# nasa/PROTEUS

Measured on AMD Instinct MI355X. Metric: Mpixels/sec DSWx classify (3660^2 7-band HLS tiles), higher is better.
Workload: dtype int16+f64

## Files before the change

### proteus_amd/csrc/dswx_outline.hip

```cpp
#include <hip/hip_runtime.h>
#include <cstdio>
#include <cstring>
#include <vector>

#include "dswx_host.h"
#include "dswx_body_rule.h"
#include "dswx_outline_rule.h"

namespace {

typedef u32x4 __attribute__((aligned(16))) out_u32x4;

constexpr int OUT_BLOCK = 256;
constexpr int OUT_PPT = 16;
constexpr int OUT_WAVES = OUT_BLOCK / 64;
constexpr int OUT_CHUNK = DSWX_OUTLINE_CHUNK;
static_assert(DSWX_OUTLINE_CHUNK == DSWX_BODY_CHUNK && DSWX_OUTLINE_SCAN_STEP == DSWX_BODY_SCAN_STEP, "the scan of the body table");
static_assert(OUT_BLOCK * OUT_PPT == OUT_CHUNK && DSWX_OUTLINE_SCAN_STEP == OUT_BLOCK, "a workgroup's threads cover a chunk");
constexpr int64_t OUT_MAX_PIXELS = 1LL << 30;
constexpr int64_t OUT_MAX_CAP = 1LL << 31;
constexpr unsigned OUT_CORNER = 0x80000000u;
constexpr int OUT_MAX_ROUNDS = 31;
constexpr unsigned OUT_NO_RING = 0xFFFFFFFFu;

struct OutlineInfo {
    unsigned long long E;
    unsigned long long R;
    unsigned ok;
    unsigned fin;
    unsigned flag[OUT_MAX_ROUNDS + 1];
};
static_assert(sizeof(OutlineInfo) <= 256, "the info block of a tile");

struct OutlineLayout {
    unsigned long long cap;
    unsigned long long base, mask, st0, st1, acc, part, info, per_tile;
    unsigned chunks_p, chunks_e, rounds, acc_blocks;
};
inline unsigned long long up16(unsigned long long v) { return (v + 15ull) & ~15ull; }
OutlineLayout outline_layout(int64_t max_edges, int64_t height, int64_t width) {
    OutlineLayout l = {};
    const unsigned long long n = (unsigned long long)(height * width);
    l.cap = (unsigned long long)max_edges < 4ull * n ? (unsigned long long)max_edges : 4ull * n;
    l.chunks_p = (unsigned)((n + OUT_CHUNK - 1) / OUT_CHUNK);
    l.chunks_e = (unsigned)((l.cap + OUT_CHUNK - 1) / OUT_CHUNK);
    while ((1ull << l.rounds) < l.cap) ++l.rounds;
    const unsigned long long rings = l.cap / 4ull;
    l.acc_blocks = (unsigned)((rings + OUT_BLOCK - 1) / OUT_BLOCK);
    unsigned long long at = 0;
    l.base = at, at += up16(4ull * n);
    l.mask = at, at += up16(n);
    l.st0 = at, at += 16ull * l.cap;
    l.st1 = at, at += 16ull * l.cap;
    l.acc = at, at += 16ull * rings;
    l.part = at, at += up16(8ull * l.chunks_e);
    l.info = at, at += 256ull;
    l.per_tile = at;
    return l;
}

struct OutlineArgs {
    const unsigned* ids;
    unsigned char* work;
    OutlineLayout l;
    unsigned long long n_elems;
    long long n_tiles;
    unsigned height, width;
    int connectivity;
    unsigned round;
    unsigned long long max_edges, max_rings;
    unsigned* chain;
    unsigned* rings;
    unsigned long long* head;
};

struct DevIds {
    const unsigned* p;
    __device__ __forceinline__ unsigned operator()(uint64_t i) const { return p[i]; }
};

__device__ __forceinline__ unsigned char* tile_work(const OutlineArgs& a, long long t) { return a.work + (unsigned long long)t * a.l.per_tile; }
__device__ __forceinline__ unsigned* w_base(const OutlineArgs& a, long long t) { return reinterpret_cast<unsigned*>(tile_work(a, t) + a.l.base); }
__device__ __forceinline__ unsigned char* w_mask(const OutlineArgs& a, long long t) { return tile_work(a, t) + a.l.mask; }
__device__ __forceinline__ out_u32x4* w_state(const OutlineArgs& a, long long t, unsigned which) {
    return reinterpret_cast<out_u32x4*>(tile_work(a, t) + (which ? a.l.st1 : a.l.st0));
}
__device__ __forceinline__ unsigned long long* w_acc(const OutlineArgs& a, long long t) {
    return reinterpret_cast<unsigned long long*>(tile_work(a, t) + a.l.acc);
}
__device__ __forceinline__ unsigned* w_part(const OutlineArgs& a, long long t) { return reinterpret_cast<unsigned*>(tile_work(a, t) + a.l.part); }
__device__ __forceinline__ OutlineInfo* w_info(const OutlineArgs& a, long long t) { return reinterpret_cast<OutlineInfo*>(tile_work(a, t) + a.l.info); }

__device__ __forceinline__ unsigned out_wave_sum(unsigned v) {
#pragma unroll
    for (int o = 32; o > 0; o >>= 1) v += __shfl_xor(v, o);
    return v;
}
__device__ __forceinline__ unsigned out_wave_scan(unsigned v, unsigned lane) {
#pragma unroll
    for (int o = 1; o < 64; o <<= 1) {
        const unsigned u = __shfl_up(v, o);
        if (lane >= (unsigned)o) v += u;
    }
    return v;
}
__device__ __forceinline__ long long out_shfl_up64(long long v, int o) {
    const unsigned lo = __shfl_up((unsigned)(unsigned long long)v, o), hi = __shfl_up((unsigned)((unsigned long long)v >> 32), o);
    return (long long)(((unsigned long long)hi << 32) | lo);
}

__device__ __forceinline__ unsigned out_block_scan(unsigned v, unsigned* wtot, unsigned* total) {
    const unsigned lane = threadIdx.x & 63u, wave = threadIdx.x >> 6;
    const unsigned inc = out_wave_scan(v, lane);
    if (lane == 63u) wtot[wave] = inc;
    __syncthreads();
    unsigned before = 0, sum = 0;
#pragma unroll
    for (int w = 0; w < OUT_WAVES; ++w) {
        if ((unsigned)w < wave) before += wtot[w];
        sum += wtot[w];
    }
    __syncthreads();
    *total = sum;
    return before + inc - v;
}

__device__ __forceinline__ unsigned out_succ_number(const OutlineArgs& a, const unsigned* ids, const unsigned* base, const unsigned char* mask,
                                                    unsigned x, unsigned y, unsigned d, unsigned v) {
    const OutlineEdge s = outline_succ(DevIds{ids}, (int64_t)x, (int64_t)y, d, (int64_t)a.width, (int64_t)a.height, v, a.connectivity);
    const unsigned long long q = (unsigned long long)s.y * a.width + (unsigned long long)s.x;
    const unsigned e = base[q] + __popc((unsigned)mask[q] & ((1u << s.d) - 1u));
    return e | (s.d != d ? OUT_CORNER : 0u);
}

__global__ __launch_bounds__(OUT_BLOCK) void dswx_outline_count_k(const OutlineArgs a) {
    __shared__ unsigned wtot[OUT_WAVES];
    const unsigned long long chunk_first = (unsigned long long)blockIdx.x * OUT_CHUNK;
    const unsigned long long first = chunk_first + (unsigned long long)threadIdx.x * OUT_PPT;
    const unsigned lane = threadIdx.x & 63u, wave = threadIdx.x >> 6;
    for (long long t = blockIdx.y; t < a.n_tiles; t += gridDim.y) {
        const unsigned* const ids = a.ids + (unsigned long long)t * a.n_elems;
        unsigned char* const mask = w_mask(a, t);
        unsigned c = 0;
        if (first < a.n_elems) {
            unsigned y = (unsigned)(first / a.width), x = (unsigned)(first - (unsigned long long)y * a.width);
            unsigned m[OUT_PPT];
#pragma unroll
            for (int i = 0; i < OUT_PPT; ++i) {
                m[i] = 0u;
                if (first + i < a.n_elems) {
                    const unsigned v = ids[first + i];
                    if (v) m[i] = outline_mask(DevIds{ids}, (int64_t)x, (int64_t)y, (int64_t)a.width, (int64_t)a.height, v);
                    c += __popc(m[i]);
                    if (++x == a.width) x = 0u, ++y;
                }
            }
            if (first + OUT_PPT <= a.n_elems) {
                u32x4 q;
#pragma unroll
                for (int w = 0; w < 4; ++w) q[w] = m[4 * w] | (m[4 * w + 1] << 8) | (m[4 * w + 2] << 16) | (m[4 * w + 3] << 24);
                *reinterpret_cast<out_u32x4*>(mask + first) = q;
            } else {
#pragma unroll
                for (int i = 0; i < OUT_PPT; ++i)
                    if (first + i < a.n_elems) mask[first + i] = (unsigned char)m[i];
            }
        }
        c = out_wave_sum(c);
        if (lane == 0) wtot[wave] = c;
        __syncthreads();
        if (threadIdx.x == 0) {
            unsigned sum = 0;
#pragma unroll
            for (int w = 0; w < OUT_WAVES; ++w) sum += wtot[w];
            w_base(a, t)[chunk_first] = sum;
        }
        __syncthreads();
    }
}

__global__ __launch_bounds__(OUT_BLOCK) void dswx_outline_scan_k(const OutlineArgs a) {
    __shared__ unsigned wtot[OUT_WAVES];
    for (long long t = blockIdx.x; t < a.n_tiles; t += gridDim.x) {
        unsigned* const b = w_base(a, t);
        unsigned long long carry = 0;
        for (unsigned first = 0; first < a.l.chunks_p; first += DSWX_OUTLINE_SCAN_STEP) {
            const unsigned c = first + threadIdx.x;
            const unsigned val = c < a.l.chunks_p ? b[(unsigned long long)c * OUT_CHUNK] : 0u;
            unsigned total;
            const unsigned before = out_block_scan(val, wtot, &total);
            if (c < a.l.chunks_p) b[(unsigned long long)c * OUT_CHUNK] = (unsigned)carry + before;
            carry += total;
        }
        OutlineInfo* const info = w_info(a, t);
        const bool ok = carry <= a.max_edges;
        if (threadIdx.x <= OUT_MAX_ROUNDS) info->flag[threadIdx.x] = 0u;
        if (threadIdx.x == 0) {
            info->E = carry;
            info->R = 0ull;
            info->ok = ok ? 1u : 0u;
            info->fin = 0u;
        }
        if (a.head && threadIdx.x < DSWX_OUTLINE_HEAD_WORDS) {
            const unsigned w = threadIdx.x;
            a.head[(unsigned long long)t * DSWX_OUTLINE_HEAD_WORDS + w] =
                w == OUTLINE_HEAD_E ? carry : w == OUTLINE_HEAD_WRITTEN ? (ok ? carry : 0ull) : w == OUTLINE_HEAD_OVERFLOW ? (ok ? 0ull : 1ull) : 0ull;
        }
    }
}

__global__ __launch_bounds__(OUT_BLOCK) void dswx_outline_base_k(const OutlineArgs a) {
    __shared__ unsigned wtot[OUT_WAVES];
    __shared__ unsigned chunk_base;
    const unsigned long long chunk_first = (unsigned long long)blockIdx.x * OUT_CHUNK;
    const unsigned long long first = chunk_first + (unsigned long long)threadIdx.x * OUT_PPT;
    for (long long t = blockIdx.y; t < a.n_tiles; t += gridDim.y) {
        if (!w_info(a, t)->ok) continue;
        unsigned* const b = w_base(a, t);
        const unsigned char* const mask = w_mask(a, t);
        unsigned m[OUT_PPT], c = 0;
#pragma unroll
        for (int i = 0; i < OUT_PPT; ++i) {
            m[i] = first + i < a.n_elems ? (unsigned)mask[first + i] : 0u;
            c += __popc(m[i]);
        }
        if (threadIdx.x == 0) chunk_base = b[chunk_first];
        unsigned total;
        const unsigned before = out_block_scan(c, wtot, &total);
        unsigned e = chunk_base + before;
#pragma unroll
        for (int i = 0; i < OUT_PPT; ++i)
            if (first + i < a.n_elems) {
                b[first + i] = e;
                e += __popc(m[i]);
            }
        __syncthreads();
    }
}

__global__ __launch_bounds__(OUT_BLOCK) void dswx_outline_emit_k(const OutlineArgs a) {
    const unsigned long long first = (unsigned long long)blockIdx.x * OUT_CHUNK + (unsigned long long)threadIdx.x * OUT_PPT;
    if (first >= a.n_elems) return;
    for (long long t = blockIdx.y; t < a.n_tiles; t += gridDim.y) {
        if (!w_info(a, t)->ok) continue;
        const unsigned* const ids = a.ids + (unsigned long long)t * a.n_elems;
        const unsigned* const b = w_base(a, t);
        const unsigned char* const mask = w_mask(a, t);
        out_u32x4* const st = w_state(a, t, 0u);
        unsigned y = (unsigned)(first / a.width), x = (unsigned)(first - (unsigned long long)y * a.width);
        for (int i = 0; i < OUT_PPT && first + i < a.n_elems; ++i) {
            const unsigned p = (unsigned)(first + i), m = mask[p];
            if (m) {
                const unsigned v = ids[p];
                unsigned e = b[p];
                for (unsigned d = 0; d < 4u; ++d)
                    if ((m >> d) & 1u) {
                        st[e] = u32x4{out_succ_number(a, ids, b, mask, x, y, d, v), e, 0u, 4u * p + d};
                        ++e;
                    }
            }
            if (++x == a.width) x = 0u, ++y;
        }
    }
}

__global__ __launch_bounds__(OUT_BLOCK) void dswx_outline_jump_k(const OutlineArgs a) {
    const unsigned long long e = (unsigned long long)blockIdx.x * OUT_BLOCK + threadIdx.x;
    const unsigned k = a.round;
    for (long long t = blockIdx.y; t < a.n_tiles; t += gridDim.y) {
        OutlineInfo* const info = w_info(a, t);
        if (!info->ok || (k > 0u && !info->flag[k - 1u])) continue;
        if ((unsigned long long)blockIdx.x * OUT_BLOCK >= info->E) continue;
        const out_u32x4* const src = w_state(a, t, k & 1u);
        out_u32x4* const dst = w_state(a, t, (k + 1u) & 1u);
        if (blockIdx.x == 0 && threadIdx.x == 0) info->fin = (k + 1u) & 1u;
        bool take = false;
        if (e < info->E) {
            const u32x4 s = src[e];
            const u32x4 o = src[s.x & ~OUT_CORNER];
            take = o.y < s.y;
            dst[e] = u32x4{(o.x & ~OUT_CORNER) | (s.x & OUT_CORNER), take ? o.y : s.y, take ? (1u << k) + o.z : s.z, s.w};
        }
        if (__any(take) && (threadIdx.x & 63u) == 0u) info->flag[k] = 1u;
    }
}

__global__ __launch_bounds__(OUT_BLOCK) void dswx_outline_ring_count_k(const OutlineArgs a) {
    __shared__ unsigned wtot[OUT_WAVES];
    const unsigned long long first = (unsigned long long)blockIdx.x * OUT_CHUNK + (unsigned long long)threadIdx.x * OUT_PPT;
    for (long long t = blockIdx.y; t < a.n_tiles; t += gridDim.y) {
        const OutlineInfo* const info = w_info(a, t);
        if (!info->ok) continue;
        const unsigned long long E = info->E;
        const out_u32x4* const st = w_state(a, t, info->fin);
        out_u32x4* const ring = w_state(a, t, info->fin ^ 1u);
        const unsigned* const ids = a.ids + (unsigned long long)t * a.n_elems;
        unsigned count = 0, length = 0;
        for (int i = 0; i < OUT_PPT && first + i < E; ++i) {
            const unsigned e = (unsigned)(first + i);
            const u32x4 s = st[e];
            if (s.y != e) continue;
            const unsigned p = s.w >> 2, d = s.w & 3u, y = p / a.width, x = p - y * a.width;
            const unsigned nx = out_succ_number(a, ids, w_base(a, t), w_mask(a, t), x, y, d, ids[p]) & ~OUT_CORNER;
            const unsigned L = st[nx].z + 1u;
            ring[e] = u32x4{L, 0u, 0u, 0u};
            ++count;
            length += L;
        }
        unsigned tc, tl;
        out_block_scan(count, wtot, &tc);
        out_block_scan(length, wtot, &tl);
        if (threadIdx.x == 0) {
            w_part(a, t)[2ull * blockIdx.x] = tc;
            w_part(a, t)[2ull * blockIdx.x + 1] = tl;
        }
    }
}

__global__ __launch_bounds__(OUT_BLOCK) void dswx_outline_ring_scan_k(const OutlineArgs a) {
    __shared__ unsigned wtot[OUT_WAVES];
    for (long long t = blockIdx.x; t < a.n_tiles; t += gridDim.x) {
        OutlineInfo* const info = w_info(a, t);
        if (!info->ok) continue;
        unsigned* const part = w_part(a, t);
        const unsigned chunks = (unsigned)((info->E + OUT_CHUNK - 1) / OUT_CHUNK);
        unsigned carry_c = 0, carry_l = 0;
        for (unsigned first = 0; first < chunks; first += DSWX_OUTLINE_SCAN_STEP) {
            const unsigned c = first + threadIdx.x;
            const unsigned vc = c < chunks ? part[2ull * c] : 0u, vl = c < chunks ? part[2ull * c + 1] : 0u;
            unsigned tc, tl;
            const unsigned bc = out_block_scan(vc, wtot, &tc), bl = out_block_scan(vl, wtot, &tl);
            if (c < chunks) part[2ull * c] = carry_c + bc, part[2ull * c + 1] = carry_l + bl;
            carry_c += tc, carry_l += tl;
        }
        if (threadIdx.x == 0) {
            info->R = carry_c;
            if (a.head) {
                a.head[(unsigned long long)t * DSWX_OUTLINE_HEAD_WORDS + OUTLINE_HEAD_R] = carry_c;
                a.head[(unsigned long long)t * DSWX_OUTLINE_HEAD_WORDS + OUTLINE_HEAD_ROWS] = carry_c < a.max_rings ? carry_c : a.max_rings;
            }
        }
    }
}

__global__ __launch_bounds__(OUT_BLOCK) void dswx_outline_ring_rank_k(const OutlineArgs a) {
    __shared__ unsigned wtot[OUT_WAVES];
    const unsigned long long first = (unsigned long long)blockIdx.x * OUT_CHUNK + (unsigned long long)threadIdx.x * OUT_PPT;
    for (long long t = blockIdx.y; t < a.n_tiles; t += gridDim.y) {
        const OutlineInfo* const info = w_info(a, t);
        if (!info->ok) continue;
        const unsigned long long E = info->E;
        const out_u32x4* const st = w_state(a, t, info->fin);
        out_u32x4* const ring = w_state(a, t, info->fin ^ 1u);
        unsigned long long* const acc = w_acc(a, t);
        const unsigned* const ids = a.ids + (unsigned long long)t * a.n_elems;
        unsigned starts = 0, count = 0, length = 0;
        for (int i = 0; i < OUT_PPT && first + i < E; ++i)
            if (st[first + i].y == (unsigned)(first + i)) {
                starts |= 1u << i;
                ++count;
                length += ring[first + i].x;
            }
        unsigned tc, tl;
        unsigned r = out_block_scan(count, wtot, &tc), o = out_block_scan(length, wtot, &tl);
        r += w_part(a, t)[2ull * blockIdx.x];
        o += w_part(a, t)[2ull * blockIdx.x + 1];
        for (int i = 0; i < OUT_PPT; ++i)
            if ((starts >> i) & 1u) {
                const unsigned e = (unsigned)(first + i), L = ring[e].x, key = st[e].w;
                ring[e] = u32x4{L, r, o, 0u};
                acc[2ull * r] = 0ull, acc[2ull * r + 1] = 0ull;
                if (a.rings && r < a.max_rings) {
                    unsigned* const row = a.rings + ((unsigned long long)t * a.max_rings + r) * DSWX_OUTLINE_ROW_WORDS;
                    row[OUTLINE_ID] = ids[key >> 2];
                    row[OUTLINE_START] = key;
                    row[OUTLINE_OFFSET] = o;
                    row[OUTLINE_LENGTH] = L;
                }
                ++r;
                o += L;
            }
    }
}

__global__ __launch_bounds__(OUT_BLOCK) void dswx_outline_scatter_k(const OutlineArgs a) {
    const unsigned long long e = (unsigned long long)blockIdx.x * OUT_BLOCK + threadIdx.x;
    const unsigned lane = threadIdx.x & 63u;
    for (long long t = blockIdx.y; t < a.n_tiles; t += gridDim.y) {
        const OutlineInfo* const info = w_info(a, t);
        if (!info->ok || (unsigned long long)blockIdx.x * OUT_BLOCK >= info->E) continue;
        const out_u32x4* const st = w_state(a, t, info->fin);
        const out_u32x4* const ring = w_state(a, t, info->fin ^ 1u);
        unsigned r = OUT_NO_RING, corners = 0;
        long long area2 = 0;
        if (e < info->E) {
            const u32x4 s = st[e];
            const u32x4 g = ring[s.y];
            r = g.y;
            if (a.chain) a.chain[(unsigned long long)t * a.max_edges + g.z + (s.z ? g.x - s.z : 0u)] = s.w;
            const unsigned p = s.w >> 2, y = p / a.width, x = p - y * a.width;
            area2 = outline_area2((int64_t)x, (int64_t)y, s.w & 3u);
            corners = s.x >> 31;
        }
        const unsigned before = __shfl_up(r, 1);
        bool head_of_run = lane == 0u || before != r;
#pragma unroll
        for (int o = 1; o < 64; o <<= 1) {
            const long long ua = out_shfl_up64(area2, o);
            const unsigned uc = __shfl_up(corners, o);
            const int uh = __shfl_up((int)head_of_run, o);
            if (lane >= (unsigned)o && !head_of_run) {
                area2 += ua;
                corners += uc;
                head_of_run = uh != 0;
            }
        }
        const unsigned after = __shfl_down(r, 1);
        if (r != OUT_NO_RING && (lane == 63u || after != r)) {
            unsigned long long* const acc = w_acc(a, t) + 2ull * r;
            if (area2) atomicAdd(acc, (unsigned long long)area2);
            if (corners) atomicAdd(acc + 1, (unsigned long long)corners);
        }
    }
}

__global__ __launch_bounds__(OUT_BLOCK) void dswx_outline_finish_k(const OutlineArgs a) {
    __shared__ unsigned wtot[OUT_WAVES];
    const unsigned long long r = (unsigned long long)blockIdx.x * OUT_BLOCK + threadIdx.x;
    for (long long t = blockIdx.y; t < a.n_tiles; t += gridDim.y) {
        const OutlineInfo* const info = w_info(a, t);
        if (!info->ok || (unsigned long long)blockIdx.x * OUT_BLOCK >= info->R) continue;
        unsigned outer = 0, holes = 0, corners = 0;
        if (r < info->R) {
            const unsigned long long* const acc = w_acc(a, t) + 2ull * r;
            const long long area2 = (long long)acc[0];
            corners = (unsigned)acc[1];
            outer = area2 > 0, holes = area2 < 0;
            if (a.rings && r < a.max_rings) {
                unsigned* const row = a.rings + ((unsigned long long)t * a.max_rings + r) * DSWX_OUTLINE_ROW_WORDS;
                row[OUTLINE_CORNERS] = corners;
                row[OUTLINE_AREA2] = (unsigned)acc[0];
                row[OUTLINE_AREA2 + 1] = (unsigned)(acc[0] >> 32);
            }
        }
        if (!a.head) continue;
        unsigned to, th, tc;
        out_block_scan(outer, wtot, &to);
        out_block_scan(holes, wtot, &th);
        out_block_scan(corners, wtot, &tc);
        if (threadIdx.x == 0) {
            unsigned long long* const head = a.head + (unsigned long long)t * DSWX_OUTLINE_HEAD_WORDS;
            if (to) atomicAdd(head + OUTLINE_HEAD_OUTER, (unsigned long long)to);
            if (th) atomicAdd(head + OUTLINE_HEAD_HOLES, (unsigned long long)th);
            if (tc) atomicAdd(head + OUTLINE_HEAD_CORNERS, (unsigned long long)tc);
        }
    }
}

struct HostIds {
    const unsigned char* p;
    inline uint32_t operator()(uint64_t i) const {
        uint32_t v;
        std::memcpy(&v, p + (size_t)i * 4, 4);
        return v;
    }
};
inline void put_u32(void* base, size_t word, uint32_t v) { std::memcpy(static_cast<unsigned char*>(base) + word * 4, &v, 4); }
inline void put_u64(void* base, size_t byte, uint64_t v) { std::memcpy(static_cast<unsigned char*>(base) + byte, &v, 8); }

int outline_check(const uint32_t* ids, const dswx_outline_spec_t* spec, int64_t n_tiles, int64_t height, int64_t width,
                  const dswx_outline_out_t* out, bool device, const void* work, uint64_t work_bytes) {
    if (!spec) return dswx_fail(DSWX_ERR_ARG, "spec is NULL");
    if (!out) return dswx_fail(DSWX_ERR_ARG, "out is NULL");
    if (spec->connectivity != 4 && spec->connectivity != 8) return dswx_fail(DSWX_ERR_ARG, "connectivity %d is neither 4 nor 8", spec->connectivity);
    if (spec->reserved != 0) return dswx_fail(DSWX_ERR_ARG, "reserved is %d, not 0", spec->reserved);
    if (n_tiles < 0 || height < 0 || width < 0 || spec->max_edges < 0 || spec->max_rings < 0) return dswx_fail(DSWX_ERR_ARG, "negative size");
    if (height > OUT_MAX_PIXELS || width > OUT_MAX_PIXELS || height * width > OUT_MAX_PIXELS)
        return dswx_fail(DSWX_ERR_ARG, "raster too large: height * width above 2^30, a key would not fit 32 bits");
    if (spec->max_edges > OUT_MAX_CAP) return dswx_fail(DSWX_ERR_ARG, "max_edges %lld above 2^31", (long long)spec->max_edges);
    if (spec->max_rings > OUT_MAX_CAP) return dswx_fail(DSWX_ERR_ARG, "max_rings %lld above 2^31", (long long)spec->max_rings);
    if (n_tiles > (1LL << 32)) return dswx_fail(DSWX_ERR_ARG, "plane too large: more than 2^32 tiles");
    if (!ids && n_tiles > 0 && height * width > 0) return dswx_fail(DSWX_ERR_ARG, "ids is NULL");
    if (!out->rings && spec->max_rings > 0) return dswx_fail(DSWX_ERR_ARG, "rings is NULL with max_rings %lld", (long long)spec->max_rings);
    if (!out->chain && out->rings) return dswx_fail(DSWX_ERR_ARG, "chain is NULL with rings wanted: a row names a place in the chain");
    if (device) {
        uint64_t need = 0;
        if (int rc = dswx_outline_work_bytes(spec, n_tiles, height, width, &need)) return rc;
        if (!work) return dswx_fail(DSWX_ERR_ARG, "work_device is NULL");
        if (work_bytes < need) return dswx_fail(DSWX_ERR_ARG, "work_bytes %llu below the %llu of dswx_outline_work_bytes", (unsigned long long)work_bytes, (unsigned long long)need);
        if (!aligned_to(ids, 4)) return dswx_fail(DSWX_ERR_ALIGN, "ids not 4-byte aligned");
        if (!aligned_to(out->chain, 4)) return dswx_fail(DSWX_ERR_ALIGN, "chain not 4-byte aligned");
        if (!aligned_to(out->rings, 4)) return dswx_fail(DSWX_ERR_ALIGN, "rings not 4-byte aligned");
        if (!aligned_to(out->head, 8)) return dswx_fail(DSWX_ERR_ALIGN, "head not 8-byte aligned");
        if (!aligned_to(work, 8)) return dswx_fail(DSWX_ERR_ALIGN, "work_device not 8-byte aligned");
    }
    return DSWX_OK;
}

}

int dswx_outline_launch(dswx_ctx* ctx, const uint32_t* ids, const dswx_outline_spec_t* spec, int64_t n_tiles, int64_t height,
                        int64_t width, const dswx_outline_out_t* out, void* work, hipStream_t s) {
    if (n_tiles == 0) {
        ctx->last_kernel = "none (empty input)";
        return DSWX_OK;
    }
    OutlineArgs a = {};
    a.ids = ids;
    a.work = reinterpret_cast<unsigned char*>((reinterpret_cast<uintptr_t>(work) + 15u) & ~(uintptr_t)15u);
    a.l = outline_layout(spec->max_edges, height, width);
    a.n_elems = (unsigned long long)(height * width);
    a.n_tiles = n_tiles;
    a.height = (unsigned)height;
    a.width = (unsigned)width;
    a.connectivity = spec->connectivity;
    a.max_edges = (unsigned long long)spec->max_edges;
    a.max_rings = (unsigned long long)spec->max_rings;
    a.chain = out->chain;
    a.rings = spec->max_rings > 0 ? out->rings : nullptr;
    a.head = reinterpret_cast<unsigned long long*>(out->head);
    const unsigned gy = (unsigned)(n_tiles < 65535 ? n_tiles : 65535);
    const dim3 block(OUT_BLOCK);
    if (a.chain && a.max_edges) HIP_TRY(hipMemsetAsync(a.chain, 0, (size_t)n_tiles * (size_t)a.max_edges * sizeof(uint32_t), s));
    if (a.rings) HIP_TRY(hipMemsetAsync(a.rings, 0, (size_t)n_tiles * (size_t)a.max_rings * DSWX_OUTLINE_ROW_WORDS * sizeof(uint32_t), s));
    if (a.l.chunks_p) hipLaunchKernelGGL(dswx_outline_count_k, dim3(a.l.chunks_p, gy), block, 0, s, a);
    hipLaunchKernelGGL(dswx_outline_scan_k, dim3(gy), block, 0, s, a);
    const unsigned edge_blocks = (unsigned)((a.l.cap + OUT_BLOCK - 1) / OUT_BLOCK);
    if (a.l.cap) {
        hipLaunchKernelGGL(dswx_outline_base_k, dim3(a.l.chunks_p, gy), block, 0, s, a);
        hipLaunchKernelGGL(dswx_outline_emit_k, dim3(a.l.chunks_p, gy), block, 0, s, a);
        for (unsigned k = 0; k < a.l.rounds; ++k) {
            a.round = k;
            hipLaunchKernelGGL(dswx_outline_jump_k, dim3(edge_blocks, gy), block, 0, s, a);
        }
        hipLaunchKernelGGL(dswx_outline_ring_count_k, dim3(a.l.chunks_e, gy), block, 0, s, a);
        hipLaunchKernelGGL(dswx_outline_ring_scan_k, dim3(gy), block, 0, s, a);
        hipLaunchKernelGGL(dswx_outline_ring_rank_k, dim3(a.l.chunks_e, gy), block, 0, s, a);
        hipLaunchKernelGGL(dswx_outline_scatter_k, dim3(edge_blocks, gy), block, 0, s, a);
        if (a.l.acc_blocks && (a.rings || a.head)) hipLaunchKernelGGL(dswx_outline_finish_k, dim3(a.l.acc_blocks, gy), block, 0, s, a);
    }
    HIP_TRY(hipGetLastError());
    char info[320];
    snprintf(info, sizeof info, "dswx_outline_count_k/base_k/emit_k grid=(%u,%u,1) block=%d chunk=%d + dswx_outline_scan_k/ring_scan_k grid=(%u,1,1) + dswx_outline_jump_k x %u and scatter_k grid=(%u,%u,1) + dswx_outline_ring_count_k/ring_rank_k grid=(%u,%u,1) + dswx_outline_finish_k grid=(%u,%u,1) connectivity=%d cap=%llu",
             a.l.chunks_p, gy, OUT_BLOCK, OUT_CHUNK, gy, a.l.cap ? a.l.rounds : 0u, edge_blocks, gy, a.l.chunks_e, gy, a.l.acc_blocks, gy, a.connectivity, a.l.cap);
    ctx->last_kernel = info;
    return DSWX_OK;
}

extern "C" {

int dswx_outline_work_bytes(const dswx_outline_spec_t* spec, int64_t n_tiles, int64_t height, int64_t width, uint64_t* bytes) {
    if (!spec) return dswx_fail(DSWX_ERR_ARG, "spec is NULL");
    if (!bytes) return dswx_fail(DSWX_ERR_ARG, "bytes is NULL");
    if (n_tiles < 0 || height < 0 || width < 0 || spec->max_edges < 0) return dswx_fail(DSWX_ERR_ARG, "negative size");
    if (height > OUT_MAX_PIXELS || width > OUT_MAX_PIXELS || height * width > OUT_MAX_PIXELS)
        return dswx_fail(DSWX_ERR_ARG, "raster too large: height * width above 2^30, a key would not fit 32 bits");
    if (spec->max_edges > OUT_MAX_CAP) return dswx_fail(DSWX_ERR_ARG, "max_edges %lld above 2^31", (long long)spec->max_edges);
    if (n_tiles > (1LL << 32)) return dswx_fail(DSWX_ERR_ARG, "plane too large: more than 2^32 tiles");
    const OutlineLayout l = outline_layout(spec->max_edges, height, width);
    if (n_tiles && l.per_tile > (1ull << 62) / (uint64_t)n_tiles) return dswx_fail(DSWX_ERR_ARG, "plane too large: the working memory would pass 2^62 bytes");
    *bytes = 16ull + (uint64_t)n_tiles * l.per_tile;
    return DSWX_OK;
}

int dswx_outline_host(const uint32_t* ids, const dswx_outline_spec_t* spec, int64_t n_tiles, int64_t height, int64_t width,
                      const dswx_outline_out_t* out) {
    if (int rc = outline_check(ids, spec, n_tiles, height, width, out, false, nullptr, 0)) return rc;
    const int64_t n = height * width, max_edges = spec->max_edges, max_rings = spec->max_rings;
    std::vector<unsigned char> todo((size_t)n);
    for (int64_t t = 0; t < n_tiles; ++t) {
        const HostIds get = {reinterpret_cast<const unsigned char*>(ids) + (size_t)t * (size_t)n * 4};
        unsigned char* const chain = out->chain ? reinterpret_cast<unsigned char*>(out->chain) + (size_t)t * (size_t)max_edges * 4 : nullptr;
        unsigned char* const rings = out->rings ? reinterpret_cast<unsigned char*>(out->rings) + (size_t)t * (size_t)max_rings * DSWX_OUTLINE_ROW_WORDS * 4 : nullptr;
        if (chain) std::memset(chain, 0, (size_t)max_edges * 4);
        if (rings) std::memset(rings, 0, (size_t)max_rings * DSWX_OUTLINE_ROW_WORDS * 4);
        uint64_t E = 0;
        for (int64_t y = 0; y < height; ++y)
            for (int64_t x = 0; x < width; ++x) {
                const uint32_t v = get((uint64_t)(y * width + x));
                const unsigned m = v ? outline_mask(get, x, y, width, height, v) : 0u;
                todo[(size_t)(y * width + x)] = (unsigned char)m;
                E += (uint64_t)__builtin_popcount(m);
            }
        uint64_t head[DSWX_OUTLINE_HEAD_WORDS] = {E, 0, 0, 0, 0, 0, 0, 0};
        if (E > (uint64_t)max_edges) head[OUTLINE_HEAD_OVERFLOW] = 1;
        else {
            uint64_t R = 0, at = 0;
            for (int64_t p = 0; p < n; ++p)
                for (unsigned d0 = 0; d0 < 4u && todo[(size_t)p]; ++d0) {
                    if (!((todo[(size_t)p] >> d0) & 1u)) continue;
                    const uint32_t v = get((uint64_t)p);
                    const uint64_t offset = at;
                    uint32_t corners = 0;
                    int64_t area2 = 0;
                    OutlineEdge e = {p % width, p / width, d0};
                    do {
                        const int64_t q = e.y * width + e.x;
                        todo[(size_t)q] = (unsigned char)(todo[(size_t)q] & ~(1u << e.d));
                        if (chain) put_u32(chain, (size_t)at, (uint32_t)(4 * q) + e.d);
                        ++at;
                        area2 += outline_area2(e.x, e.y, e.d);
                        const OutlineEdge f = outline_succ(get, e.x, e.y, e.d, width, height, v, spec->connectivity);
                        corners += f.d != e.d;
                        e = f;
                    } while ((e.y * width + e.x != p || e.d != d0) && at < E);
                    if (rings && R < (uint64_t)max_rings) {
                        unsigned char* const row = rings + (size_t)R * DSWX_OUTLINE_ROW_WORDS * 4;
                        put_u32(row, OUTLINE_ID, v);
                        put_u32(row, OUTLINE_START, (uint32_t)(4 * p) + d0);
                        put_u32(row, OUTLINE_OFFSET, (uint32_t)offset);
                        put_u32(row, OUTLINE_LENGTH, (uint32_t)(at - offset));
                        put_u32(row, OUTLINE_CORNERS, corners);
                        put_u64(row, OUTLINE_AREA2 * 4, (uint64_t)area2);
                    }
                    ++R;
                    head[OUTLINE_HEAD_OUTER] += area2 > 0;
                    head[OUTLINE_HEAD_HOLES] += area2 < 0;
                    head[OUTLINE_HEAD_CORNERS] += corners;
                }
            head[OUTLINE_HEAD_R] = R;
            head[OUTLINE_HEAD_ROWS] = R < (uint64_t)max_rings ? R : (uint64_t)max_rings;
            head[OUTLINE_HEAD_WRITTEN] = E;
        }
        if (out->head)
            for (int w = 0; w < DSWX_OUTLINE_HEAD_WORDS; ++w) put_u64(out->head, (size_t)(t * DSWX_OUTLINE_HEAD_WORDS + w) * 8, head[w]);
    }
    return DSWX_OK;
}

int dswx_outline_device(dswx_ctx_t* ctx, const uint32_t* ids, const dswx_outline_spec_t* spec, int64_t n_tiles, int64_t height,
                        int64_t width, const dswx_outline_out_t* out, void* work_device, uint64_t work_bytes, void* stream) {
    if (int rc = outline_check(ids, spec, n_tiles, height, width, out, true, work_device, work_bytes)) return rc;
    if (!ctx) return dswx_fail(DSWX_ERR_ARG, "ctx is NULL");
    HIP_TRY(hipSetDevice(ctx->device));
    return dswx_outline_launch(ctx, ids, spec, n_tiles, height, width, out, work_device, dswx_stream_of(ctx, stream));
}

}
```

### proteus_amd/csrc/dswx_outline_rule.h

```cpp
#pragma once
#include <cstdint>

#include "dswx_hip.h"

namespace {

constexpr int DSWX_OUTLINE_CHUNK = 4096;
constexpr int DSWX_OUTLINE_SCAN_STEP = 256;

constexpr int OUTLINE_ID = 0, OUTLINE_START = 1, OUTLINE_OFFSET = 2, OUTLINE_LENGTH = 3, OUTLINE_CORNERS = 4, OUTLINE_AREA2 = 6;
constexpr int OUTLINE_HEAD_E = 0, OUTLINE_HEAD_R = 1, OUTLINE_HEAD_ROWS = 2, OUTLINE_HEAD_WRITTEN = 3, OUTLINE_HEAD_OUTER = 4,
              OUTLINE_HEAD_HOLES = 5, OUTLINE_HEAD_CORNERS = 6, OUTLINE_HEAD_OVERFLOW = 7;

__host__ __device__ __forceinline__ int outline_tx(unsigned d) { return (d == 0u) - (d == 2u); }
__host__ __device__ __forceinline__ int outline_ty(unsigned d) { return (d == 1u) - (d == 3u); }
__host__ __device__ __forceinline__ int outline_ox(unsigned d) { return outline_ty(d); }
__host__ __device__ __forceinline__ int outline_oy(unsigned d) { return -outline_tx(d); }

template <typename Ids>
__host__ __device__ __forceinline__ bool outline_same(const Ids& ids, int64_t x, int64_t y, int64_t width, int64_t height, uint32_t v) {
    return x >= 0 && y >= 0 && x < width && y < height && ids((uint64_t)(y * width + x)) == v;
}

template <typename Ids>
__host__ __device__ __forceinline__ unsigned outline_mask(const Ids& ids, int64_t x, int64_t y, int64_t width, int64_t height, uint32_t v) {
    unsigned m = 0;
#pragma unroll
    for (unsigned d = 0; d < 4u; ++d)
        if (!outline_same(ids, x + outline_ox(d), y + outline_oy(d), width, height, v)) m |= 1u << d;
    return m;
}

struct OutlineEdge {
    int64_t x, y;
    unsigned d;
};
template <typename Ids>
__host__ __device__ __forceinline__ OutlineEdge outline_succ(const Ids& ids, int64_t x, int64_t y, unsigned d, int64_t width,
                                                             int64_t height, uint32_t v, int connectivity) {
    const int64_t ax = x + outline_tx(d), ay = y + outline_ty(d);
    const int64_t bx = ax + outline_ox(d), by = ay + outline_oy(d);
    const bool a = outline_same(ids, ax, ay, width, height, v), b = outline_same(ids, bx, by, width, height, v);
    const OutlineEdge right = {x, y, (d + 1u) & 3u}, straight = {ax, ay, d}, left = {bx, by, (d + 3u) & 3u};
    if (connectivity == 4) return !a ? right : !b ? straight : left;
    return b ? left : a ? straight : right;
}

__host__ __device__ __forceinline__ int64_t outline_area2(int64_t x, int64_t y, unsigned d) {
    return d == 0u ? -y : d == 1u ? x + 1 : d == 2u ? y + 1 : -x;
}

}
```

Baseline: 306,700.

## Store outline edge prefix per 16-pixel unit and vectorize mask neighbour loads

The per-pixel edge-number base table becomes one prefix per 16-pixel unit. Edge numbers are rebuilt from the unit prefix plus popcounts over the unit's 16 mask bytes, which cuts base-table writes and memory footprint. The count kernel now loads ids in 4-wide vector runs, takes horizontal neighbours by wave shuffles, and skips up/down loads for all-zero runs. The emit kernel skips units with no edges and walks only the set mask bytes. In exchange, every successor lookup does an extra 16-byte mask load plus popcount arithmetic, and the indexing has more edge cases.

```diff
diff --git a/proteus_amd/csrc/dswx_outline.hip b/proteus_amd/csrc/dswx_outline.hip
--- a/proteus_amd/csrc/dswx_outline.hip
+++ b/proteus_amd/csrc/dswx_outline.hip
@@ -10,9 +10,13 @@
 namespace {
 
 typedef u32x4 __attribute__((aligned(16))) out_u32x4;
+typedef u32x4 __attribute__((aligned(4))) out_u32x4_w;
 
 constexpr int OUT_BLOCK = 256;
 constexpr int OUT_PPT = 16;
+constexpr int OUT_RUN = 4;
+constexpr int OUT_RUNS = OUT_PPT / OUT_RUN;
+static_assert(OUT_PPT == (int)DSWX_OUTLINE_UNIT, "a thread of launches 3 and 4 owns a unit");
 constexpr int OUT_WAVES = OUT_BLOCK / 64;
 constexpr int OUT_CHUNK = DSWX_OUTLINE_CHUNK;
 static_assert(DSWX_OUTLINE_CHUNK == DSWX_BODY_CHUNK && DSWX_OUTLINE_SCAN_STEP == DSWX_BODY_SCAN_STEP, "the scan of the body table");
@@ -48,7 +52,7 @@
     const unsigned long long rings = l.cap / 4ull;
     l.acc_blocks = (unsigned)((rings + OUT_BLOCK - 1) / OUT_BLOCK);
     unsigned long long at = 0;
-    l.base = at, at += up16(4ull * n);
+    l.base = at, at += up16(4ull * ((n + DSWX_OUTLINE_UNIT - 1) / DSWX_OUTLINE_UNIT));
     l.mask = at, at += up16(n);
     l.st0 = at, at += 16ull * l.cap;
     l.st1 = at, at += 16ull * l.cap;
@@ -125,55 +129,103 @@
     return before + inc - v;
 }
 
-__device__ __forceinline__ unsigned out_succ_number(const OutlineArgs& a, const unsigned* ids, const unsigned* base, const unsigned char* mask,
-                                                    unsigned x, unsigned y, unsigned d, unsigned v) {
+struct OutUnit {
+    unsigned first, prefix;
+    uint64_t lo, hi;
+};
+__device__ __forceinline__ unsigned out_succ_number(const OutlineArgs& a, const unsigned* ids, const unsigned* prefix, const unsigned char* mask,
+                                                    unsigned x, unsigned y, unsigned d, unsigned v, const OutUnit& own) {
     const OutlineEdge s = outline_succ(DevIds{ids}, (int64_t)x, (int64_t)y, d, (int64_t)a.width, (int64_t)a.height, v, a.connectivity);
-    const unsigned long long q = (unsigned long long)s.y * a.width + (unsigned long long)s.x;
-    const unsigned e = base[q] + __popc((unsigned)mask[q] & ((1u << s.d) - 1u));
+    const unsigned q = (unsigned)s.y * a.width + (unsigned)s.x;
+    const unsigned first = q & ~(DSWX_OUTLINE_UNIT - 1u), pos = q & (DSWX_OUTLINE_UNIT - 1u);
+    unsigned e;
+    if (first == own.first) e = outline_edge_number(own.prefix, own.lo, own.hi, pos, s.d);
+    else {
+        const u32x4 w = *reinterpret_cast<const out_u32x4*>(mask + first);
+        e = outline_edge_number(prefix[q / DSWX_OUTLINE_UNIT], (uint64_t)w.x | ((uint64_t)w.y << 32), (uint64_t)w.z | ((uint64_t)w.w << 32), pos, s.d);
+    }
     return e | (s.d != d ? OUT_CORNER : 0u);
+}
+
+__device__ __forceinline__ void out_unit_masks(const unsigned char* mask, unsigned long long first, unsigned long long n, uint64_t& lo, uint64_t& hi) {
+    const u32x4 w = *reinterpret_cast<const out_u32x4*>(mask + first);
+    lo = (uint64_t)w.x | ((uint64_t)w.y << 32), hi = (uint64_t)w.z | ((uint64_t)w.w << 32);
+    const unsigned long long rest = n - first;
+    if (rest < 8ull) lo &= (1ull << (8u * (unsigned)rest)) - 1ull;
+    if (rest <= 8ull) hi = 0ull;
+    else if (rest < 16ull) hi &= (1ull << (8u * (unsigned)(rest - 8ull))) - 1ull;
+}
+
+__device__ __forceinline__ void out_load_run(const unsigned* ids, long long first, long long shift, bool whole, long long n, uint32_t (&c)[OUT_RUN]) {
+    if (whole) {
+        const u32x4 w = *reinterpret_cast<const out_u32x4_w*>(ids + (first + shift));
+        c[0] = w.x, c[1] = w.y, c[2] = w.z, c[3] = w.w;
+    } else {
+#pragma unroll
+        for (int i = 0; i < OUT_RUN; ++i) {
+            const long long p = first + i, q = p + shift;
+            c[i] = p < n && q >= 0 && q < n ? ids[q] : 0u;
+        }
+    }
 }
 
 __global__ __launch_bounds__(OUT_BLOCK) void dswx_outline_count_k(const OutlineArgs a) {
     __shared__ unsigned wtot[OUT_WAVES];
+    const unsigned lane = threadIdx.x & 63u, wave = threadIdx.x >> 6;
     const unsigned long long chunk_first = (unsigned long long)blockIdx.x * OUT_CHUNK;
-    const unsigned long long first = chunk_first + (unsigned long long)threadIdx.x * OUT_PPT;
-    const unsigned lane = threadIdx.x & 63u, wave = threadIdx.x >> 6;
+    const long long first = (long long)(chunk_first + (unsigned long long)threadIdx.x * OUT_PPT);
+    const long long n = (long long)a.n_elems;
     for (long long t = blockIdx.y; t < a.n_tiles; t += gridDim.y) {
         const unsigned* const ids = a.ids + (unsigned long long)t * a.n_elems;
         unsigned char* const mask = w_mask(a, t);
-        unsigned c = 0;
-        if (first < a.n_elems) {
-            unsigned y = (unsigned)(first / a.width), x = (unsigned)(first - (unsigned long long)y * a.width);
-            unsigned m[OUT_PPT];
-#pragma unroll
-            for (int i = 0; i < OUT_PPT; ++i) {
-                m[i] = 0u;
-                if (first + i < a.n_elems) {
-                    const unsigned v = ids[first + i];
-                    if (v) m[i] = outline_mask(DevIds{ids}, (int64_t)x, (int64_t)y, (int64_t)a.width, (int64_t)a.height, v);
-                    c += __popc(m[i]);
-                    if (++x == a.width) x = 0u, ++y;
-                }
-            }
-            if (first + OUT_PPT <= a.n_elems) {
-                u32x4 q;
-#pragma unroll
-                for (int w = 0; w < 4; ++w) q[w] = m[4 * w] | (m[4 * w + 1] << 8) | (m[4 * w + 2] << 16) | (m[4 * w + 3] << 24);
-                *reinterpret_cast<out_u32x4*>(mask + first) = q;
-            } else {
-#pragma unroll
-                for (int i = 0; i < OUT_PPT; ++i)
-                    if (first + i < a.n_elems) mask[first + i] = (unsigned char)m[i];
-            }
-        }
-        c = out_wave_sum(c);
-        if (lane == 0) wtot[wave] = c;
+        OutlineRun r[OUT_RUNS];
+        uint32_t c[OUT_RUNS][OUT_RUN];
+#pragma unroll
+        for (int j = 0; j < OUT_RUNS; ++j) {
+            r[j] = outline_run((uint64_t)(first + OUT_RUN * j), OUT_RUN, a.n_elems, a.width);
+            out_load_run(ids, first + OUT_RUN * j, 0, r[j].whole, n, c[j]);
+        }
+        uint32_t before = __shfl_up(c[OUT_RUNS - 1][OUT_RUN - 1], 1), after = __shfl_down(c[0][0], 1);
+        if (lane == 0u) before = r[0].before ? ids[first - 1] : 0u;
+        if (lane == 63u) after = r[OUT_RUNS - 1].after ? ids[first + OUT_PPT] : 0u;
+        uint32_t up[OUT_RUNS][OUT_RUN], down[OUT_RUNS][OUT_RUN];
+        bool any[OUT_RUNS];
+#pragma unroll
+        for (int j = 0; j < OUT_RUNS; ++j) {
+            any[j] = (c[j][0] | c[j][1] | c[j][2] | c[j][3]) != 0u;
+            if (any[j]) {
+                out_load_run(ids, first + OUT_RUN * j, -(long long)a.width, r[j].up, n, up[j]);
+                out_load_run(ids, first + OUT_RUN * j, (long long)a.width, r[j].down, n, down[j]);
+            }
+        }
+        unsigned mw[OUT_RUNS], count = 0;
+#pragma unroll
+        for (int j = 0; j < OUT_RUNS; ++j) {
+            mw[j] = 0u;
+            if (any[j]) {
+                unsigned m[OUT_RUN];
+                const unsigned x = (unsigned)(first + OUT_RUN * j) % a.width;
+                outline_run_masks<OUT_RUN>(c[j], up[j], down[j], j > 0 ? c[j > 0 ? j - 1 : j][OUT_RUN - 1] : before,
+                                           j + 1 < OUT_RUNS ? c[j + 1 < OUT_RUNS ? j + 1 : j][0] : after, (uint64_t)(first + OUT_RUN * j), x, a.n_elems,
+                                           a.width, m);
+                mw[j] = m[0] | (m[1] << 8) | (m[2] << 16) | (m[3] << 24);
+                count += __popc(mw[j]);
+            }
+        }
+        if (first + OUT_PPT <= n) *reinterpret_cast<out_u32x4*>(mask + first) = u32x4{mw[0], mw[1], mw[2], mw[3]};
+        else {
+#pragma unroll
+            for (int i = 0; i < OUT_PPT; ++i)
+                if (first + i < n) mask[first + i] = (unsigned char)(mw[i / OUT_RUN] >> (8 * (i % OUT_RUN)));
+        }
+        count = out_wave_sum(count);
+        if (lane == 0) wtot[wave] = count;
         __syncthreads();
         if (threadIdx.x == 0) {
             unsigned sum = 0;
 #pragma unroll
             for (int w = 0; w < OUT_WAVES; ++w) sum += wtot[w];
-            w_base(a, t)[chunk_first] = sum;
+            w_base(a, t)[chunk_first / DSWX_OUTLINE_UNIT] = sum;
         }
         __syncthreads();
     }
@@ -181,15 +233,16 @@
 
 __global__ __launch_bounds__(OUT_BLOCK) void dswx_outline_scan_k(const OutlineArgs a) {
     __shared__ unsigned wtot[OUT_WAVES];
+    constexpr unsigned long long STRIDE = OUT_CHUNK / DSWX_OUTLINE_UNIT;
     for (long long t = blockIdx.x; t < a.n_tiles; t += gridDim.x) {
         unsigned* const b = w_base(a, t);
         unsigned long long carry = 0;
         for (unsigned first = 0; first < a.l.chunks_p; first += DSWX_OUTLINE_SCAN_STEP) {
             const unsigned c = first + threadIdx.x;
-            const unsigned val = c < a.l.chunks_p ? b[(unsigned long long)c * OUT_CHUNK] : 0u;
+            const unsigned val = c < a.l.chunks_p ? b[c * STRIDE] : 0u;
             unsigned total;
             const unsigned before = out_block_scan(val, wtot, &total);
-            if (c < a.l.chunks_p) b[(unsigned long long)c * OUT_CHUNK] = (unsigned)carry + before;
+            if (c < a.l.chunks_p) b[c * STRIDE] = (unsigned)carry + before;
             carry += total;
         }
         OutlineInfo* const info = w_info(a, t);
@@ -217,23 +270,16 @@
     for (long long t = blockIdx.y; t < a.n_tiles; t += gridDim.y) {
         if (!w_info(a, t)->ok) continue;
         unsigned* const b = w_base(a, t);
-        const unsigned char* const mask = w_mask(a, t);
-        unsigned m[OUT_PPT], c = 0;
-#pragma unroll
-        for (int i = 0; i < OUT_PPT; ++i) {
-            m[i] = first + i < a.n_elems ? (unsigned)mask[first + i] : 0u;
-            c += __popc(m[i]);
-        }
-        if (threadIdx.x == 0) chunk_base = b[chunk_first];
+        unsigned c = 0;
+        if (first < a.n_elems) {
+            uint64_t lo, hi;
+            out_unit_masks(w_mask(a, t), first, a.n_elems, lo, hi);
+            c = (unsigned)(__popcll(lo) + __popcll(hi));
+        }
+        if (threadIdx.x == 0) chunk_base = b[chunk_first / DSWX_OUTLINE_UNIT];
         unsigned total;
         const unsigned before = out_block_scan(c, wtot, &total);
-        unsigned e = chunk_base + before;
-#pragma unroll
-        for (int i = 0; i < OUT_PPT; ++i)
-            if (first + i < a.n_elems) {
-                b[first + i] = e;
-                e += __popc(m[i]);
-            }
+        if (first < a.n_elems) b[first / DSWX_OUTLINE_UNIT] = chunk_base + before;
         __syncthreads();
     }
 }
@@ -243,23 +289,31 @@
     if (first >= a.n_elems) return;
     for (long long t = blockIdx.y; t < a.n_tiles; t += gridDim.y) {
         if (!w_info(a, t)->ok) continue;
+        const unsigned char* const mask = w_mask(a, t);
+        OutUnit own;
+        out_unit_masks(mask, first, a.n_elems, own.lo, own.hi);
+        if (!(own.lo | own.hi)) continue;
         const unsigned* const ids = a.ids + (unsigned long long)t * a.n_elems;
         const unsigned* const b = w_base(a, t);
-        const unsigned char* const mask = w_mask(a, t);
         out_u32x4* const st = w_state(a, t, 0u);
-        unsigned y = (unsigned)(first / a.width), x = (unsigned)(first - (unsigned long long)y * a.width);
-        for (int i = 0; i < OUT_PPT && first + i < a.n_elems; ++i) {
-            const unsigned p = (unsigned)(first + i), m = mask[p];
-            if (m) {
-                const unsigned v = ids[p];
-                unsigned e = b[p];
+        own.first = (unsigned)first;
+        own.prefix = b[first / DSWX_OUTLINE_UNIT];
+        unsigned e = own.prefix;
+        unsigned y = (unsigned)first / a.width, x = (unsigned)first - y * a.width, at = 0;
+        for (int h = 0; h < 2; ++h) {
+            uint64_t w = h ? own.hi : own.lo;
+            while (w) {
+                const unsigned byte = (unsigned)__builtin_ctzll(w) >> 3, i = 8u * h + byte, m = (unsigned)(w >> (8u * byte)) & 0xFFu;
+                w &= ~(0xFFull << (8u * byte));
+                for (; at < i; ++at)
+                    if (++x == a.width) x = 0u, ++y;
+                const unsigned p = (unsigned)first + i, v = ids[p];
                 for (unsigned d = 0; d < 4u; ++d)
                     if ((m >> d) & 1u) {
-                        st[e] = u32x4{out_succ_number(a, ids, b, mask, x, y, d, v), e, 0u, 4u * p + d};
+                        st[e] = u32x4{out_succ_number(a, ids, b, mask, x, y, d, v, own), e, 0u, 4u * p + d};
                         ++e;
                     }
             }
-            if (++x == a.width) x = 0u, ++y;
         }
     }
 }
@@ -301,7 +355,7 @@
             const u32x4 s = st[e];
             if (s.y != e) continue;
             const unsigned p = s.w >> 2, d = s.w & 3u, y = p / a.width, x = p - y * a.width;
-            const unsigned nx = out_succ_number(a, ids, w_base(a, t), w_mask(a, t), x, y, d, ids[p]) & ~OUT_CORNER;
+            const unsigned nx = out_succ_number(a, ids, w_base(a, t), w_mask(a, t), x, y, d, ids[p], OutUnit{~0u, 0u, 0ull, 0ull}) & ~OUT_CORNER;
             const unsigned L = st[nx].z + 1u;
             ring[e] = u32x4{L, 0u, 0u, 0u};
             ++count;
diff --git a/proteus_amd/csrc/dswx_outline_rule.h b/proteus_amd/csrc/dswx_outline_rule.h
--- a/proteus_amd/csrc/dswx_outline_rule.h
+++ b/proteus_amd/csrc/dswx_outline_rule.h
@@ -22,13 +22,60 @@
     return x >= 0 && y >= 0 && x < width && y < height && ids((uint64_t)(y * width + x)) == v;
 }
 
-template <typename Ids>
-__host__ __device__ __forceinline__ unsigned outline_mask(const Ids& ids, int64_t x, int64_t y, int64_t width, int64_t height, uint32_t v) {
+__host__ __device__ __forceinline__ unsigned outline_mask_of(uint32_t v, const uint32_t (&nb)[4], const bool (&has)[4]) {
     unsigned m = 0;
 #pragma unroll
     for (unsigned d = 0; d < 4u; ++d)
-        if (!outline_same(ids, x + outline_ox(d), y + outline_oy(d), width, height, v)) m |= 1u << d;
+        if (!(has[d] && nb[d] == v)) m |= 1u << d;
     return m;
+}
+
+template <typename Ids>
+__host__ __device__ __forceinline__ unsigned outline_mask(const Ids& ids, int64_t x, int64_t y, int64_t width, int64_t height, uint32_t v) {
+    uint32_t nb[4];
+    bool has[4];
+#pragma unroll
+    for (unsigned d = 0; d < 4u; ++d) {
+        const int64_t nx = x + outline_ox(d), ny = y + outline_oy(d);
+        has[d] = nx >= 0 && ny >= 0 && nx < width && ny < height;
+        nb[d] = has[d] ? ids((uint64_t)(ny * width + nx)) : 0u;
+    }
+    return outline_mask_of(v, nb, has);
+}
+
+struct OutlineRun {
+    bool whole, up, down, before, after;
+};
+__host__ __device__ __forceinline__ OutlineRun outline_run(uint64_t first, unsigned U, uint64_t n, uint64_t width) {
+    OutlineRun r;
+    r.whole = first + U <= n;
+    r.up = r.whole && first >= width;
+    r.down = first + U + width <= n;
+    r.before = first > 0 && first <= n;
+    r.after = first + U < n;
+    return r;
+}
+
+template <int U>
+__host__ __device__ __forceinline__ void outline_run_masks(const uint32_t (&c)[U], const uint32_t (&up)[U], const uint32_t (&down)[U], uint32_t before,
+                                                           uint32_t after, uint64_t first, uint32_t x, uint64_t n, uint32_t width, unsigned (&m)[U]) {
+#pragma unroll
+    for (int i = 0; i < U; ++i) {
+        const uint64_t p = first + (uint64_t)i;
+        const uint32_t nb[4] = {up[i], i + 1 < U ? c[i + 1 < U ? i + 1 : i] : after, down[i], i > 0 ? c[i > 0 ? i - 1 : i] : before};
+        const bool has[4] = {p >= width, x + 1u < width, p + width < n, x > 0u};
+        m[i] = c[i] != 0u && p < n ? outline_mask_of(c[i], nb, has) : 0u;
+        if (++x == width) x = 0u;
+    }
+}
+
+constexpr unsigned DSWX_OUTLINE_UNIT = 16;
+__host__ __device__ __forceinline__ unsigned outline_edge_number(unsigned prefix, uint64_t lo, uint64_t hi, unsigned pos, unsigned d) {
+    const unsigned shift = 8u * (pos & 7u);
+    const uint64_t word = pos < 8u ? lo : hi;
+    const unsigned below = (pos < 8u ? 0u : (unsigned)__builtin_popcountll(lo)) + (unsigned)__builtin_popcountll(word & ((1ull << shift) - 1ull));
+    const unsigned own = (unsigned)(word >> shift) & 0xFFu;
+    return prefix + below + (unsigned)__builtin_popcount(own & ((1u << d) - 1u));
 }
 
 struct OutlineEdge {
```

Result: no change. 306,000 (-0.2%).
